# a1q123456/image_stitching

Hardware: AMD Instinct MI355X
Metric: 4K frames stitched/sec (higher is better)
Workload: dtype u8

## Files before the change

### image_stitching_amd/csrc/homography.h

```cpp
#pragma once
#include "common.h"

struct HomoCall {
    const float* src;
    const float* dst;
    uint8_t* mask;
    long long pt_off;
    int n;
    int active;
};

struct HomoResult {
    double H[9];
    int ok;
    int iters;
    int ninl;
    int pad;
};

struct HomoBatch {
    int count = 0;
    long long points = 0;
    int max_iters = 0;
    void* mem = nullptr;
    size_t bytes = 0;
    HomoCall* calls = nullptr;
    HomoResult* results = nullptr;
    void* state = nullptr;
    int* sub_idx = nullptr;
    double* Hc = nullptr;
    int* valid = nullptr;
    int* good = nullptr;
    float* scr = nullptr;
    double* rec = nullptr;
    int* draw_idx = nullptr;
    int* fin = nullptr;
    int2* work = nullptr;
    unsigned* work_ctr = nullptr;
};

int homo_batch_reserve(MisContext* ctx, HomoBatch* b, int count, long long points, int max_iters);
int homo_batch_debug_states(MisContext* ctx, const HomoBatch* b, int* out, int cap);
void homo_batch_release(HomoBatch* b);
enum MotionModel { MODEL_HOMOGRAPHY = 0, MODEL_AFFINE_PARTIAL = 1 };
struct HomoParams { double thresh; int max_iters; double confidence; MotionModel model = MODEL_HOMOGRAPHY; int refine_iters = 10; };
struct HomoHooks {
    hipEvent_t after_first_draw = nullptr, after_second_draw = nullptr;
    hipStream_t spec_stream = nullptr;
    hipEvent_t spec_fork = nullptr, spec_join = nullptr, spec_mark = nullptr;
};
enum RansacPhase { PHASE_FIRST = 0, PHASE_SECOND = 1 };
enum TailStep { TAIL_MASK, TAIL_REFINE };
int homo_solve(MisContext* ctx, HomoBatch* b, const HomoParams& prm, hipStream_t stream = nullptr, const HomoHooks* hooks = nullptr);
int homo_phase(MisContext* ctx, HomoBatch* b, const HomoParams& prm, RansacPhase phase, hipStream_t stream, const HomoHooks* hooks = nullptr);
int homo_tails(MisContext* ctx, HomoBatch* b, const HomoParams& prm, RansacPhase phase, TailStep step, hipStream_t stream);
```

### image_stitching_amd/csrc/homography.hip

```cpp
#include "homography.h"
#include "dev_math.h"
#include <algorithm>
#include <mutex>
#include <vector>

namespace {

#ifndef MIS_PHASE0
#define MIS_PHASE0 128
#endif
constexpr int PHASE0 = MIS_PHASE0;
constexpr int RNG_TABLE = 1 << 17;
#ifndef MIS_HQ_HYPS
#define MIS_HQ_HYPS 64
#endif
constexpr int HQ_HYPS = MIS_HQ_HYPS;
constexpr int TB = 256;

struct RansacState {
    int mode;
    int n_sub;
    int iter, niters, max_good, done, best_k;
    int tail_pending;
    int draw_k, draw_fail;
    long long draw_pos;
    int spec_k, spec_fail;
    long long spec_pos;
};
__device__ __forceinline__ void ransac_reset(RansacState* st, const int mode, const int max_iters) {
    st->mode = mode;
    st->n_sub = 0; st->iter = 0; st->niters = max_iters > 1 ? max_iters : 1; st->max_good = 0; st->done = 0; st->best_k = -1; st->tail_pending = 0;
    st->draw_k = 0; st->draw_fail = 0; st->draw_pos = 0;
    st->spec_k = 0; st->spec_fail = 0; st->spec_pos = 0;
}

enum DrawPhase { DRAW_FIRST, DRAW_SECOND, DRAW_SPEC };
enum TailKind {
    TAIL_REPLAY_FINISH,
    TAIL_REPLAY_ONLY,
    TAIL_MASK_ONLY,
    TAIL_REFINE_ONLY,
};

#ifdef MIS_TAIL_PROF
#define PROF_ONLY(...) __VA_ARGS__
__device__ unsigned long long g_draw_prof[12];
__device__ unsigned long long g_hyp_prof[8];
__device__ unsigned long long g_jac_prof[8];
__device__ unsigned long long g_tail_log[6 * 1024];
__device__ unsigned g_tail_log_n;
__device__ unsigned long long g_tail_prof[12];
#else
#define PROF_ONLY(...)
#endif
#if defined(MIS_TAIL_PROF) && defined(MIS_JAC_PROF)
#define JAC_ONLY(...) __VA_ARGS__
#else
#define JAC_ONLY(...)
#endif
#if defined(MIS_TAIL_PROF) && defined(MIS_PS_PROF)
#define PS_ONLY(...) __VA_ARGS__
#else
#define PS_ONLY(...)
#endif
#define PROF_T0(v) PROF_ONLY(unsigned long long v = wall_clock64())
#define PROF_ADD(i, v) PROF_ONLY(do { if (threadIdx.x == 0) atomicAdd(&g_tail_prof[i], wall_clock64() - (v)); } while (0))
#define JP_T(v) JAC_ONLY(const unsigned long long v = __builtin_readcyclecounter())
#define JP_ADD(i, a, b) JAC_ONLY(do { if (threadIdx.x == 0) atomicAdd(&g_jac_prof[i], (b) - (a)); } while (0))
#define JP_KEEP(...) JAC_ONLY(asm volatile("" :: __VA_ARGS__))
#define PS_T(v) PS_ONLY(const unsigned long long v = __builtin_readcyclecounter())
#define PS_SUM(v) PS_ONLY(unsigned long long v = 0)
#define PS_ACC(v, a, b) PS_ONLY(v += (b) - (a))
#define PS_KEEP(x) PS_ONLY(asm volatile("" :: "v"(x)))
#define PS_ADD(i, who, a, b) PS_ONLY(do { if (threadIdx.x == (who)) atomicAdd(&g_jac_prof[i], (b) - (a)); } while (0))
#define PROF_ROTATIONS(S, n) PROF_ONLY(do { if (threadIdx.x == 0) { atomicAdd(&g_tail_prof[1], (unsigned long long)(n)); (S).prof_rot += (n); } } while (0))
#define PROF_LM_ITERATION(S) PROF_ONLY(do { if (threadIdx.x == 0) { atomicAdd(&g_tail_prof[3], 1ull); (S).prof_lm++; } } while (0))
#define PROF_LM_PASS(np) PROF_ONLY(do { if (threadIdx.x == 0) { atomicAdd(&g_jac_prof[6], (unsigned long long)(np)); atomicAdd(&g_jac_prof[7], 1ull); } } while (0))
#define PROF_FIRST_ENTRY(kind, want, wg_in) PROF_ONLY(const unsigned long long wg_in = wall_clock64(); if ((kind) == TAIL_REFINE_ONLY && (want) == 0 && threadIdx.x == 0) atomicMin(&g_tail_prof[8], wg_in))
#define PROF_LAST_EXIT(kind, want, wg_in) PROF_ONLY(do { if ((kind) == TAIL_REFINE_ONLY && (want) == 0 && threadIdx.x == 0) { const unsigned long long o = wall_clock64(); \
        atomicMax(&g_tail_prof[9], o); atomicMax(&g_tail_prof[10], o - (wg_in)); atomicAdd(&g_tail_prof[11], 1ull); } } while (0))
#define PROF_REPLAY(lo, t0) PROF_ONLY(do { if ((lo) > 0) { const unsigned long long d = wall_clock64() - (t0); atomicAdd(&g_hyp_prof[6], d); atomicMax(&g_hyp_prof[7], d); } } while (0))
#define PROF_TAIL_BEGIN(S, pt) PROF_ONLY(unsigned long long pt = wall_clock64(); if (threadIdx.x == 0) { (S).prof_rot = 0; (S).prof_lm = 0; })
#define PROF_TAIL_END(S, np, kind, want, pt) PROF_ONLY(do { if (threadIdx.x == 0) { \
        atomicAdd(&g_tail_prof[5], wall_clock64() - (pt)); atomicAdd(&g_tail_prof[6], 1ull); atomicMax(&g_tail_prof[7], wall_clock64() - (pt)); \
        const int code[4] = {0, 1, 3, 4}; const unsigned k = atomicAdd(&g_tail_log_n, 1u); if (k < 1024) { unsigned long long* e = g_tail_log + 6 * k; e[0] = np; e[1] = (S).prof_lm; e[2] = (S).prof_rot; e[3] = wall_clock64() - (pt); e[4] = code[kind] * 10 + (want); e[5] = pt; } } } while (0))
struct DrawProf {
    PROF_ONLY(unsigned long long t0 = wall_clock64(), last = t0, sim, dbl; int chunks = 0;)
    __device__ __forceinline__ void simulated() { PROF_ONLY(chunks++; sim = wall_clock64();) }
    __device__ __forceinline__ void doubled() { PROF_ONLY(dbl = wall_clock64();) }
    __device__ __forceinline__ void ranked() {
        PROF_ONLY(const unsigned long long now = wall_clock64(); atomicAdd(&g_draw_prof[8], sim - last); atomicAdd(&g_draw_prof[9], dbl - sim); atomicAdd(&g_draw_prof[10], now - dbl); atomicAdd(&g_draw_prof[11], 1ull);)
    }
    __device__ __forceinline__ void chunk_end() { PROF_ONLY(last = wall_clock64();) }
// ... 604 lines not shown
            for (int i = 0; i < n; i++) { double tv = s.e(HQ_V + n * m + i); s.e(HQ_V + n * m + i) = s.e(HQ_V + n * k + i); s.e(HQ_V + n * k + i) = tv; }
        }
        __builtin_amdgcn_fence(__ATOMIC_ACQ_REL, "wavefront");
    }
}

__device__ int dlt4_quad(const float* M, const float* m, const QSlot s, const int q, double* H) {
    const int count = 4;
    double cMx = 0, cMy = 0, cmx = 0, cmy = 0, sMx = 0, sMy = 0, smx = 0, smy = 0;
    for (int i = 0; i < count; i++) { cmx += m[2 * i]; cmy += m[2 * i + 1]; cMx += M[2 * i]; cMy += M[2 * i + 1]; }
    cmx /= count; cmy /= count; cMx /= count; cMy /= count;
    for (int i = 0; i < count; i++) {
        smx += fabs(m[2 * i] - cmx); smy += fabs(m[2 * i + 1] - cmy);
        sMx += fabs(M[2 * i] - cMx); sMy += fabs(M[2 * i + 1] - cMy);
    }
    if (fabs(smx) < DBL_EPSILON || fabs(smy) < DBL_EPSILON || fabs(sMx) < DBL_EPSILON || fabs(sMy) < DBL_EPSILON) return 0;
    smx = count / smx; smy = count / smy; sMx = count / sMx; sMy = count / sMy;
    double LtL[45];
#pragma unroll
    for (int e = 0; e < 45; e++) LtL[e] = 0;
#pragma unroll
    for (int i = 0; i < count; i++) {
        const double x = (m[2 * i] - cmx) * smx, y = (m[2 * i + 1] - cmy) * smy;
        const double X = (M[2 * i] - cMx) * sMx, Y = (M[2 * i + 1] - cMy) * sMy;
        const double Lx[9] = {X, Y, 1, 0, 0, 0, -x * X, -x * Y, -x};
        const double Ly[9] = {0, 0, 0, X, Y, 1, -y * X, -y * Y, -y};
        int e = 0;
#pragma unroll
        for (int j = 0; j < 9; j++)
#pragma unroll
            for (int k = j; k < 9; k++, e++) LtL[e] += Lx[j] * Lx[k] + Ly[j] * Ly[k];
    }
    {
        int e = 0;
#pragma unroll
        for (int j = 0; j < 9; j++)
#pragma unroll
            for (int k = j; k < 9; k++, e++) {
                if ((e & 3) != q) continue;
                if (k == j) s.e(HQ_W + j) = LtL[e];
                else s.e(hq_T(j) + k) = LtL[e];
            }
    }
    __builtin_amdgcn_fence(__ATOMIC_ACQ_REL, "wavefront");
    jacobi9_quad(s, q);
    double H0[9];
    for (int i = 0; i < 9; i++) H0[i] = s.e(HQ_V + 72 + i);
    const double nrm[8] = {cmx, cmy, cMx, cMy, smx, smy, sMx, sMy};
    dlt_denormalise(H0, nrm, H);
    return 1;
}

constexpr int HQ_WG_PER_CU = 2;
constexpr int HC_WG_PER_CU = 4;
constexpr int HC_HYPS = 4;
enum { WL_N = 0, WL_SOLVE = 1, WL_CTRS = 2 };
static_assert(HQ_HYPS % 16 == 0 && HQ_HYPS % HC_HYPS == 0, "a work-list entry splits into whole solve and count tickets");
__device__ __forceinline__ unsigned first_ticket() { return __builtin_amdgcn_readfirstlane(blockIdx.x * (blockDim.x >> 6) + (threadIdx.x >> 6)); }
__device__ __forceinline__ unsigned next_ticket(unsigned* ctr, unsigned tickets) {
    const unsigned waves = gridDim.x * (blockDim.x >> 6);
    if (tickets <= waves) return tickets;
    return waves + __builtin_amdgcn_readfirstlane(atomicAdd(ctr, (threadIdx.x & 63) == 0 ? 1u : 0u));
}

__global__ __launch_bounds__(4 * HQ_HYPS) void hyp_quad_kernel(const HomoCall* calls, const RansacState* states, const int* sub_idx, double* Hc, int* valid,
                                                               int max_iters, const int2* work, unsigned* work_ctr) {
#if MIS_CHAIN_PRIO
    __builtin_amdgcn_s_setprio(MIS_CHAIN_PRIO);
#endif
    extern __shared__ double sl[];
    const int lane = threadIdx.x & 63, q = lane & 3;
    const int h = threadIdx.x >> 2;
    const unsigned tickets = work_ctr[WL_N] * (HQ_HYPS / 16);
    const QSlot s{sl + h};
    for (unsigned tk = first_ticket(); tk < tickets; tk = next_ticket(work_ctr + WL_SOLVE, tickets)) {
        const int2 w = work[tk / (HQ_HYPS / 16)];
        const int b = w.x;
        const RansacState& st = states[b];
        const int limit = min(st.n_sub, st.niters);
        const int k = w.y + (int)(tk % (HQ_HYPS / 16)) * 16 + (lane >> 2);
        if (k < limit) {
            const HomoCall c = calls[b];
            const int* id = sub_idx + ((size_t)b * max_iters + k) * 4;
            float ms1[8], ms2[8];
#pragma unroll
            for (int i = 0; i < 4; i++) {
                int qq = id[i];
                ms1[2 * i] = c.src[2 * qq]; ms1[2 * i + 1] = c.src[2 * qq + 1];
                ms2[2 * i] = c.dst[2 * qq]; ms2[2 * i + 1] = c.dst[2 * qq + 1];
            }
            double H[9];
            const int ok = dlt4_quad(ms1, ms2, s, q, H);
            if (ok) {
                double* o = Hc + ((size_t)b * max_iters + k) * 9;
#pragma unroll
                for (int i = 0; i < 9; i++) o[i] = H[i];
            }
            valid[(size_t)b * max_iters + k] = ok;
        }
    }
}

constexpr int HC_UNROLL = 4;
__global__ __launch_bounds__(256) void hyp_count_kernel(const HomoCall* calls, const RansacState* states, const double* Hc, const int* valid, int* good,
                                                        int max_iters, float thr, const int2* work, const unsigned* work_ctr) {
    const int lane = threadIdx.x & 63;
    const unsigned tickets = work_ctr[WL_N] * (HQ_HYPS / HC_HYPS), waves = gridDim.x * (blockDim.x >> 6);
    for (unsigned tk = first_ticket(); tk < tickets; tk += waves) {
        const int2 w = work[tk / (HQ_HYPS / HC_HYPS)];
        const int b = w.x;
        const RansacState& st = states[b];
        const int limit = min(st.n_sub, st.niters);
        const int k0 = w.y + (int)(tk % (HQ_HYPS / HC_HYPS)) * HC_HYPS;
        if (k0 >= limit) continue;
        const size_t e0 = (size_t)b * max_iters + k0;
        float Hf[HC_HYPS][9];
        bool use[HC_HYPS];
        int cnt[HC_HYPS];
#pragma unroll
        for (int j = 0; j < HC_HYPS; j++) {
            use[j] = k0 + j < limit && valid[e0 + j];
            cnt[j] = 0;
#pragma unroll
            for (int i = 0; i < 9; i++) Hf[j][i] = use[j] ? (float)Hc[(e0 + j) * 9 + i] : 0.f;
        }
        const HomoCall c = calls[b];
        const float2* src = reinterpret_cast<const float2*>(c.src);
        const float2* dst = reinterpret_cast<const float2*>(c.dst);
        for (int i0 = 0; i0 < c.n; i0 += 64 * HC_UNROLL) {
            float2 M[HC_UNROLL], m[HC_UNROLL];
            bool in[HC_UNROLL];
#pragma unroll
            for (int u = 0; u < HC_UNROLL; u++) {
                const int i = i0 + 64 * u + lane;
                in[u] = i < c.n;
                M[u] = src[min(i, c.n - 1)]; m[u] = dst[min(i, c.n - 1)];
            }
#pragma unroll
            for (int u = 0; u < HC_UNROLL; u++)
#pragma unroll
                for (int j = 0; j < HC_HYPS; j++)
                    if (use[j]) cnt[j] += __popcll(__ballot(in[u] && is_inlier(Hf[j], M[u].x, M[u].y, m[u].x, m[u].y, thr)));
        }
#pragma unroll
        for (int j = 0; j < HC_HYPS; j++) if (k0 + j < limit) good[e0 + j] = cnt[j];
    }
}

#ifndef MIS_PS_PTS
#define MIS_PS_PTS 32
#endif
constexpr int PS_PTS = MIS_PS_PTS;
constexpr int PS_TERMS = 42;
constexpr int PS_PITCH = 43;
constexpr int PS_STAGE = PS_PTS * PS_PITCH;
constexpr size_t TAIL_DYN_LDS = sizeof(double) * 2 * PS_STAGE;
struct TailShared {
    double A[81], V[81], W[9];
    double best[9], nrm[8];
    double lm[8 + 8 + 64 + 64 + 8 + 8 + 8 + 8];
    float Hf[9];
    int indR[9], indC[9];
    int np, go;
    int bad;
    double chunk[TB * 10];
    int staged;
    int done_now;
    int base, wcnt[TB / 64];
    PROF_ONLY(int prof_rot, prof_lm;)
};
__device__ __forceinline__ float4 tail_load_point(const float* s1, const float* d1, int i) {
    const float2 dd = reinterpret_cast<const float2*>(d1)[i], ss = reinterpret_cast<const float2*>(s1)[i];
    return make_float4(dd.x, dd.y, ss.x, ss.y);
}
__device__ __forceinline__ void lds_barrier() { mis_lds_barrier(); }

__device__ __forceinline__ void wave_sync() {
    __builtin_amdgcn_fence(__ATOMIC_ACQ_REL, "wavefront");
    __builtin_amdgcn_wave_barrier();
}
__device__ __forceinline__ double jc_readlane(double v, int lane) {
    return __hiloint2double(__builtin_amdgcn_readlane(__double2hiint(v), lane), __builtin_amdgcn_readlane(__double2loint(v), lane));
}
template <int CTRL, int ROW_MASK = 0xf>
__device__ __forceinline__ double jc_max_step(double v) {
    const int hi = __double2hiint(v), lo = __double2loint(v);
    const int ohi = ROW_MASK == 0xf ? 0 : hi, olo = ROW_MASK == 0xf ? 0 : lo;
    const double o = __hiloint2double(__builtin_amdgcn_update_dpp(ohi, hi, CTRL, ROW_MASK, 0xf, false), __builtin_amdgcn_update_dpp(olo, lo, CTRL, ROW_MASK, 0xf, false));
    double r;
    asm("v_max_f64 %0, %1, %2" : "=v"(r) : "v"(v), "v"(o));
    return r;
}
__device__ __forceinline__ double jc_row_max(double v) {
    v = jc_max_step<0xB1>(v);
    v = jc_max_step<0x4E>(v);
    v = jc_max_step<0x141>(v);
    v = jc_max_step<0x140>(v);
    return v;
// ... 605 lines not shown
template <bool AFFINE = false>
__device__ __forceinline__ void mask_and_compact(TailShared& S, const TailProblem& p, const float thr) {
    const int t = threadIdx.x, n = p.n;
    const HomoCall& c = p.c;
    for (int i0 = 0; i0 < n; i0 += TB) {
        int i = i0 + t, f = 0;
        if (i < n) f = AFFINE ? aff_is_inlier(S.Hf, c.src[2 * i], c.src[2 * i + 1], c.dst[2 * i], c.dst[2 * i + 1], thr)
                              : is_inlier(S.Hf, c.src[2 * i], c.src[2 * i + 1], c.dst[2 * i], c.dst[2 * i + 1], thr);
        if (c.mask && i < n) c.mask[i] = (uint8_t)f;
        unsigned long long bal = __ballot(f);
        int within = __popcll(bal & ((1ull << (t & 63)) - 1ull));
        if ((t & 63) == 0) S.wcnt[t >> 6] = __popcll(bal);
        __syncthreads();
        int off = S.base;
        for (int k = 0; k < (t >> 6); k++) off += S.wcnt[k];
        if (f) {
            p.s1[2 * (off + within)] = c.src[2 * i]; p.s1[2 * (off + within) + 1] = c.src[2 * i + 1];
            p.d1[2 * (off + within)] = c.dst[2 * i]; p.d1[2 * (off + within) + 1] = c.dst[2 * i + 1];
        }
        __syncthreads();
        if (t == 0) { int s = 0; for (int k = 0; k < TB / 64; k++) s += S.wcnt[k]; S.base += s; }
        __syncthreads();
    }
}

__device__ __forceinline__ void refine_on_inliers(TailShared& S, const TailProblem& p, const int np, const TailKind kind, const int want) {
    const int t = threadIdx.x;
    PROF_TAIL_BEGIN(S, pt);
    if (np > 0) {
        const float4 pt0 = t < np ? tail_load_point(p.s1, p.d1, t) : make_float4(0.f, 0.f, 0.f, 0.f);
        dlt_coop(S, p.s1, p.d1, np, pt0, p.rec);
        PROF_ADD(4, pt);
        lm_refine_coop(S, p.s1, p.d1, np, pt0, p.rec);
    }
    PROF_TAIL_END(S, np, kind, want, pt);
}

template <class Model>
__device__ __forceinline__ void tail_problem(TailShared& S, const Model& m, const HomoCall* calls, RansacState* states, const int* valid, const int* good, float* scr_all,
                                             HomoResult* results, int lo, int hi, int max_iters, double confidence, float thr, int* fin, TailKind kind, int want, unsigned* work_ctr) {
    if (work_ctr && blockIdx.x == 0 && threadIdx.x < WL_CTRS) work_ctr[threadIdx.x] = 0;
#if MIS_CHAIN_PRIO
    __builtin_amdgcn_s_setprio(MIS_CHAIN_PRIO);
#endif
    if (threadIdx.x == 0) { S.staged = m.staged; S.bad = 0; }
    m.reset_stages();
    __syncthreads();
    const int b = blockIdx.x, t = threadIdx.x;
    TailProblem p;
    p.b = b; p.c = calls[b]; p.n = p.c.n; p.st = states + b; p.res = results + b;
    p.s1 = scr_all + 4 * p.c.pt_off; p.d1 = p.s1 + 2 * (size_t)(p.n > 0 ? p.n : 0); p.rec = m.rec(p.c);
    RansacState* const st = p.st;
    const bool refines = kind == TAIL_REFINE_ONLY;
    if (kind == TAIL_MASK_ONLY || refines) {
        if (st->tail_pending != (refines ? 2 : 1) || fin[b] != want) return;
        __syncthreads();
    } else {
        if (st->done) return;
        const int mode = st->mode;
        if (t == 0) S.done_now = 0;
        __syncthreads();
        if (mode != 2) { m.no_loop(S, p, mode, lo, fin); return; }
        replay_hypotheses<Model::MODEL_POINTS>(S, p, valid, good, lo, hi, max_iters, confidence, fin);
        __syncthreads();
        if (!S.done_now) return;
        if (kind == TAIL_REPLAY_ONLY) { if (t == 0) st->tail_pending = 1; return; }
    }
    const int result = st->max_good > 0;
    if (!refines && t == 0) { p.res->iters = st->iter; p.res->ok = result; p.res->ninl = 0; }
    if (!result) {
        for (int i = t; p.c.mask && i < p.n; i += TB) p.c.mask[i] = 0;
        if (t == 0) st->tail_pending = 0;
        return;
    }
    if (t == 0) { m.load_best(S, p, max_iters); S.base = refines ? p.res->ninl : 0; }
    __syncthreads();
    if (!refines) mask_and_compact<Model::AFFINE>(S, p, thr);
    const int np = S.base;
    if (kind == TAIL_MASK_ONLY) {
        if (t == 0) { p.res->ninl = np; m.store(p.res, S.best); st->tail_pending = 2; }
        return;
    }
    m.refine(S, p, np, kind, want);
    if (t == 0) { m.store(p.res, S.best); p.res->ninl = np; if (refines) st->tail_pending = 0; }
}

struct HomographyTail {
    static constexpr int MODEL_POINTS = 4;
    static constexpr bool AFFINE = false;
    const double* Hc; double* rec_all; int staged;
    PROF_ONLY(unsigned long long wg_in;)
    __device__ __forceinline__ void reset_stages() const {
        if (staged)
            for (int i = threadIdx.x; i < 2 * PS_PTS; i += TB) tail_dyn[i * PS_PITCH + PS_TERMS] = 0.;
    }
    __device__ __forceinline__ double* rec(const HomoCall& c) const { return rec_all + 10 * c.pt_off; }
    __device__ __forceinline__ void no_loop(TailShared& S, const TailProblem& p, const int mode, const int lo, int* fin) const { finish_without_loop(S, p, mode, lo, fin); }
    __device__ __forceinline__ void load_best(TailShared& S, const TailProblem& p, const int max_iters) const {
        const double* hb = Hc + ((size_t)p.b * max_iters + p.st->best_k) * 9;
        for (int i = 0; i < 9; i++) { S.best[i] = hb[i]; S.Hf[i] = (float)hb[i]; }
    }
    __device__ __forceinline__ void refine(TailShared& S, const TailProblem& p, const int np, const TailKind kind, const int want) const {
        refine_on_inliers(S, p, np, kind, want);
        PROF_LAST_EXIT(kind, want, wg_in);
    }
    __device__ __forceinline__ void store(HomoResult* res, const double* best) const { for (int i = 0; i < 9; i++) res->H[i] = best[i]; }
};
__global__ __launch_bounds__(TB) __attribute__((amdgpu_waves_per_eu(MIS_TAIL_WAVES, 8))) void scan_tail_kernel(const HomoCall* calls, RansacState* states, const double* Hc, const int* valid, const int* good,
                                                       float* scr_all, double* rec_all, HomoResult* results, int lo, int hi, int max_iters,
                                                       double confidence, float thr, int* fin, TailKind kind, int want, int staged, unsigned* work_ctr) {
    PROF_FIRST_ENTRY(kind, want, wg_in);
    __shared__ TailShared S;
    tail_problem(S, HomographyTail{Hc, rec_all, staged PROF_ONLY(, wg_in)}, calls, states, valid, good, scr_all, results, lo, hi, max_iters, confidence, thr, fin, kind, want, work_ctr);
}


__device__ __forceinline__ void aff_hypothesis(const float2 p1, const float2 P1, const float2 p2, const float2 P2, double* M) {
    const double x1 = p1.x, y1 = p1.y, X1 = P1.x, Y1 = P1.y, x2 = p2.x, y2 = p2.y, X2 = P2.x, Y2 = P2.y;
    const double d = 1. / ((x1 - x2) * (x1 - x2) + (y1 - y2) * (y1 - y2));
    const double S0 = d * ((X1 - X2) * (x1 - x2) + (Y1 - Y2) * (y1 - y2));
    const double S1 = d * ((Y1 - Y2) * (x1 - x2) - (X1 - X2) * (y1 - y2));
    const double S2 = d * ((Y1 - Y2) * (x1 * y2 - x2 * y1) - (X1 * y2 - X2 * y1) * (y1 - y2) - (X1 * x2 - X2 * x1) * (x1 - x2));
    const double S3 = d * (-(X1 - X2) * (x1 * y2 - x2 * y1) - (Y1 * x2 - Y2 * x1) * (x1 - x2) - (Y1 * y2 - Y2 * y1) * (y1 - y2));
    M[0] = S0; M[1] = -S1; M[2] = S2; M[3] = S1; M[4] = S0; M[5] = S3;
}
__device__ __forceinline__ void aff_hypothesis_of(const HomoCall& c, const int* id, double* M) {
    const float2* src = reinterpret_cast<const float2*>(c.src);
    const float2* dst = reinterpret_cast<const float2*>(c.dst);
    aff_hypothesis(src[id[0]], dst[id[0]], src[id[1]], dst[id[1]], M);
}

constexpr int AD_CHUNK = 4096;
constexpr int AD_PER = AD_CHUNK / TB;
// ... 328 lines not shown
    }
    return n;
}

void homo_batch_release(HomoBatch* b) {
    if (b->mem) hipFree(b->mem);
    b->mem = nullptr; b->bytes = 0;
}

namespace {

struct Engine {
    MisContext* ctx; HomoBatch* b; hipStream_t st; RngTable rt; HomoHooks hk;
    int max_iters, p0; double confidence; float thr;
    bool affine; int lm_iters;
    static constexpr size_t hq_lds = sizeof(double) * HQ_ELEMS * HQ_STRIDE;

    int open(MisContext* ctx_, HomoBatch* b_, const HomoParams& prm, hipStream_t stream, const HomoHooks* hooks) {
        ctx = ctx_; b = b_; hk = hooks ? *hooks : HomoHooks();
        MIS_CHECK(ctx, prm.max_iters >= 1 && prm.max_iters <= b->max_iters, MIS_E_INVALID, "max_iters %d outside the reserved range", prm.max_iters);
        MIS_CHECK(ctx, prm.confidence > 0 && prm.confidence < 1, MIS_E_INVALID, "confidence must be in (0,1)");
        MIS_CHECK(ctx, prm.model == MODEL_HOMOGRAPHY || prm.model == MODEL_AFFINE_PARTIAL, MIS_E_UNSUPPORTED, "unknown motion model %d", (int)prm.model);
        MIS_CHECK(ctx, prm.refine_iters >= 0, MIS_E_INVALID, "refine_iters must be >= 0");
        affine = prm.model == MODEL_AFFINE_PARTIAL; lm_iters = prm.refine_iters;
        if (int rc = rng_table(ctx, &rt); rc != MIS_OK) return rc;
        const double thresh = prm.thresh <= 0 ? 3 : prm.thresh;
        thr = (float)(thresh * thresh);
        max_iters = prm.max_iters; p0 = std::min(PHASE0, max_iters); confidence = prm.confidence;
        st = stream ? stream : ctx->stream;
        static bool attr_set[64] = {false};
        if (!attr_set[ctx->device & 63]) {
            MIS_HIP(ctx, hipFuncSetAttribute((const void*)hyp_quad_kernel, hipFuncAttributeMaxDynamicSharedMemorySize, (int)hq_lds));
            attr_set[ctx->device & 63] = true;
        }
        return MIS_OK;
    }
    int close(int rc) const { if (rc == MIS_OK) MIS_HIP(ctx, hipGetLastError()); return rc; }
    void draw(DrawPhase phase, hipStream_t s) const {
        if (affine) {
            hipLaunchKernelGGL(aff_draw_kernel, dim3(b->count), dim3(TB), 0, s, b->calls, (RansacState*)b->state, b->sub_idx, rt.U, rt.state_T, max_iters, phase,
                               phase == DRAW_FIRST ? p0 : max_iters, b->work, b->work_ctr);
            return;
        }
        hipLaunchKernelGGL(draw_kernel, dim3(b->count), dim3(DRAW_TB), 0, s, b->calls, (RansacState*)b->state, b->sub_idx, b->draw_idx, rt.U, rt.state_T, max_iters, phase,
                           phase == DRAW_FIRST ? p0 : max_iters, b->work, b->work_ctr, confidence);
    }
    void hypotheses() const {
        const int ncu = std::max(ctx->num_cu, 1);
        if (affine) {
            hipLaunchKernelGGL(aff_score_kernel, dim3(AH_WG_PER_CU * ncu), dim3(256), 0, st, b->calls, (RansacState*)b->state, (const int*)b->sub_idx, b->valid, b->good,
                               max_iters, thr, (const int2*)b->work, (const unsigned*)b->work_ctr);
            return;
        }
        hipLaunchKernelGGL(hyp_quad_kernel, dim3(HQ_WG_PER_CU * ncu), dim3(4 * HQ_HYPS), hq_lds, st, b->calls, (RansacState*)b->state, b->sub_idx, b->Hc, b->valid, max_iters,
                           (const int2*)b->work, b->work_ctr);
        hipLaunchKernelGGL(hyp_count_kernel, dim3(HC_WG_PER_CU * ncu), dim3(256), 0, st, b->calls, (RansacState*)b->state, (const double*)b->Hc, (const int*)b->valid, b->good,
                           max_iters, thr, (const int2*)b->work, b->work_ctr);
    }
    void scan_tail(TailKind kind, RansacPhase phase) const {
        static const bool plain = getenv("MIS_TAIL_PLAIN") != nullptr && atoi(getenv("MIS_TAIL_PLAIN")) != 0;
        const int staged = (kind == TAIL_REPLAY_ONLY || kind == TAIL_MASK_ONLY || plain) ? 0 : 1;
        const bool replay = kind == TAIL_REPLAY_FINISH || kind == TAIL_REPLAY_ONLY, second = phase == PHASE_SECOND;
        const int lo = replay && second ? p0 : 0, hi = replay && second ? max_iters : p0, want = !replay && second ? 1 : 0;
        if (affine) {
            hipLaunchKernelGGL(aff_tail_kernel, dim3(b->count), dim3(TB), 0, st, b->calls, (RansacState*)b->state, (const int*)b->sub_idx, (const int*)b->valid,
                               (const int*)b->good, b->scr, b->results, lo, hi, max_iters, confidence, thr, b->fin, kind, want, lm_iters, replay ? b->work_ctr : nullptr);
            return;
        }
        hipLaunchKernelGGL(scan_tail_kernel, dim3(b->count), dim3(TB), staged ? TAIL_DYN_LDS : (size_t)0, st, b->calls, (RansacState*)b->state, b->Hc, b->valid, b->good, b->scr,
                           b->rec, b->results, lo, hi, max_iters, confidence, thr, b->fin, kind, want, staged, replay ? b->work_ctr : nullptr);
    }
    int run_phase(RansacPhase ph, TailKind replay) const {
        if (ph == PHASE_FIRST) {
            MIS_HIP(ctx, hipMemsetAsync(b->fin, 0xff, sizeof(int) * (size_t)b->count, st));
            draw(DRAW_FIRST, st);
            if (hk.after_first_draw) MIS_HIP(ctx, hipEventRecord(hk.after_first_draw, st));
            if (hk.spec_stream && max_iters > p0 && !affine) {
                MIS_HIP(ctx, hipEventRecord(hk.spec_fork, st));
                MIS_HIP(ctx, hipStreamWaitEvent(hk.spec_stream, hk.spec_fork, 0));
                draw(DRAW_SPEC, hk.spec_stream);
                MIS_HIP(ctx, hipEventRecord(hk.spec_join, hk.spec_stream));
                if (hk.spec_mark) MIS_HIP(ctx, hipEventRecord(hk.spec_mark, hk.spec_stream));
            }
        } else {
            if (max_iters <= p0) return MIS_OK;
            if (hk.spec_stream && !affine) MIS_HIP(ctx, hipStreamWaitEvent(st, hk.spec_join, 0));
            draw(DRAW_SECOND, st);
            if (hk.after_second_draw) MIS_HIP(ctx, hipEventRecord(hk.after_second_draw, st));
        }
        hypotheses();
        scan_tail(replay, ph);
        return MIS_OK;
    }
};

}

int homo_solve(MisContext* ctx, HomoBatch* b, const HomoParams& prm, hipStream_t stream, const HomoHooks* hooks) {
    Engine e;
    int rc = e.open(ctx, b, prm, stream, hooks);
    if (rc == MIS_OK) rc = e.run_phase(PHASE_FIRST, TAIL_REPLAY_FINISH);
    if (rc == MIS_OK) rc = e.run_phase(PHASE_SECOND, TAIL_REPLAY_FINISH);
    return e.close(rc);
}

int homo_phase(MisContext* ctx, HomoBatch* b, const HomoParams& prm, RansacPhase phase, hipStream_t stream, const HomoHooks* hooks) {
    Engine e;
    int rc = e.open(ctx, b, prm, stream, hooks);
    if (rc == MIS_OK) rc = e.run_phase(phase, TAIL_REPLAY_ONLY);
    return e.close(rc);
}

int homo_tails(MisContext* ctx, HomoBatch* b, const HomoParams& prm, RansacPhase phase, TailStep step, hipStream_t stream) {
    Engine e;
    const int rc = e.open(ctx, b, prm, stream, nullptr);
    if (rc == MIS_OK) e.scan_tail(step == TAIL_MASK ? TAIL_MASK_ONLY : TAIL_REFINE_ONLY, phase);
    return e.close(rc);
}
```

### image_stitching_amd/csrc/match.hip

```cpp
#include "common.h"
#include <thread>
#include <chrono>
#include <atomic>
#include "dev_math.h"
#include "homography.h"
#include <algorithm>
#include <vector>

namespace {

struct FeatDev {
    const uint8_t* desc;
    const MisKeyPoint* kps;
    int n, w, h;
};

#include "knn_plan.h"

constexpr int KNN_TILE = 256;
__global__ __launch_bounds__(256) void knn2_hamming_kernel(const FeatDev* feats, const PairDesc* pairs, int* idx2, float* dist2) {
    __shared__ uint4 tr[KNN_TILE * 2];
    const PairDesc pd = pairs[blockIdx.y >> 1];
    const bool fwd = (blockIdx.y & 1) == 0;
    const FeatDev Q = feats[fwd ? pd.i : pd.j], T = feats[fwd ? pd.j : pd.i];
// ... 732 lines not shown
};
int carve_pinned(MisContext* ctx, Arena& arena, const MatchPlan& pl, MatchPinned* h) {
    const size_t n = pl.fd.size(), np = pl.pairs.size(), mt = pl.m_total;
    auto lay = [&](Carver c) {
        h->feats = (FeatDev*)c.at(sizeof(FeatDev) * n); h->pairs = (PairDesc*)c.at(sizeof(PairDesc) * np); h->frames = (HmFrame*)c.at(sizeof(HmFrame) * n);
        h->jobs = (HmJob*)c.at(sizeof(HmJob) * pl.hm_jobs.size()); h->nm = (int*)c.at(sizeof(int) * np); h->out = (PairOut*)c.at(sizeof(PairOut) * np);
        h->r1 = (HomoResult*)c.at(sizeof(HomoResult) * np); h->r2 = (HomoResult*)c.at(sizeof(HomoResult) * np); h->r3 = (HomoResult*)c.at(sizeof(HomoResult) * np);
        h->fin = (int*)c.at(sizeof(int) * np); h->m = (MisDMatch*)c.at(sizeof(MisDMatch) * mt); h->mask = (uint8_t*)c.at(mt); h->l2_bad = (volatile int*)c.at(sizeof(int));
        return c.off;
    };
    MIS_HIP(ctx, arena.reserve(lay(Carver{})));
    lay(Carver{(uintptr_t)arena.p});
    return MIS_OK;
}

int enqueue_knn(MisContext* ctx, MatchWorkspace* ws, const MatchPlan& pl, const MisFeatures* feats, const MatchDev& d, const MatchPinned& h) {
    hipStream_t st = ctx->stream;
    const int n = (int)pl.fd.size(), np = (int)pl.pairs.size();
    if (pl.kind == DESC_L2) return l2_knn2_pairs(ctx, ws->l2, feats, n, pl.pairs.data(), np, true, d.idx, d.dist, (int*)h.l2_bad);
    if (pl.maxq > HM_MAX_TRAINS) {
        hipLaunchKernelGGL(knn2_hamming_kernel, dim3((pl.maxq + 255) / 256, 2 * np), dim3(256), 0, st, (const FeatDev*)d.feats, (const PairDesc*)d.pairs, d.idx, d.dist);
        return MIS_OK;
    }
    Carver lc;
    const size_t o_fr = lc.take(sizeof(HmFrame) * n), o_jobs = lc.take(sizeof(HmJob) * pl.hm_jobs.size());
    for (int i = 0; i < n; i++) {
        const size_t rows = (size_t)(std::max(feats[i].n, 1) + HM_ROWPAD - 1) / HM_ROWPAD * HM_ROWPAD;
        h.frames[i].train_off = lc.take(rows * 128); h.frames[i].query_off = lc.take(rows * 128);
    }
    MIS_HIP(ctx, ws->l2.reserve(lc.off));
    uint8_t* L = (uint8_t*)ws->l2.p;
    MIS_HIP(ctx, hipMemcpyAsync(L + o_fr, h.frames, sizeof(HmFrame) * n, hipMemcpyHostToDevice, st));
    const int maxpad = (pl.maxq + HM_ROWPAD - 1) / HM_ROWPAD * HM_ROWPAD;
    hipLaunchKernelGGL(hamming_expand4_kernel, dim3(maxpad * 8 / 256, n), dim3(256), 0, st, (const FeatDev*)d.feats, (const HmFrame*)(L + o_fr), (int8_t*)L);
    memcpy(h.jobs, pl.hm_jobs.data(), sizeof(HmJob) * pl.hm_jobs.size());
    MIS_HIP(ctx, hipMemcpyAsync(L + o_jobs, h.jobs, sizeof(HmJob) * pl.hm_jobs.size(), hipMemcpyHostToDevice, st));
    hipLaunchKernelGGL(knn2_hamming_fp4_kernel, dim3((unsigned)pl.hm_jobs.size()), dim3(256), 0, st, (const FeatDev*)d.feats, (const PairDesc*)d.pairs,
                       (const HmFrame*)(L + o_fr), (const int8_t*)L, d.idx, d.dist, (const HmJob*)(L + o_jobs));
    return MIS_OK;
}

int enqueue_chains(MisContext* ctx, MatchWorkspace* ws, int np, const MisMatchParams* p, int model, const MatchDev& d, const MatchPinned& h) {
    hipStream_t st = ctx->stream;
    int rc;
    if (!ws->side && (rc = mis_aux_stream(ctx, 0, &ws->side)) != MIS_OK) return rc;
    trace_mark(ws, 0, st);
    if (!ws->third && (rc = mis_aux_stream(ctx, 1, &ws->third)) != MIS_OK) return rc;
    MIS_HIP(ctx, hipEventRecord(ws->ev_matches.ev, st));
    MIS_HIP(ctx, hipStreamWaitEvent(ws->third, ws->ev_matches.ev, 0));
    hipLaunchKernelGGL(pack_lists_kernel, dim3(np), dim3(256), 0, ws->third, (const PairDesc*)d.pairs, np, (const int*)d.nm, (const MisDMatch*)d.matches, h.m, h.nm);
    MIS_HIP(ctx, hipEventRecord(ws->ev_lists.ev, ws->third));
    if (model == MIS_MATCH_AFFINE_PARTIAL) {
        const HomoParams aprm{p->ransac_thresh, p->max_iters, p->confidence, MODEL_AFFINE_PARTIAL, 10};
        for (RansacPhase ph : {PHASE_FIRST, PHASE_SECOND})
            if ((rc = homo_phase(ctx, &ws->b1, aprm, ph, st)) != MIS_OK || (rc = homo_tails(ctx, &ws->b1, aprm, ph, TAIL_MASK, st)) != MIS_OK ||
                (rc = homo_tails(ctx, &ws->b1, aprm, ph, TAIL_REFINE, st)) != MIS_OK) return rc;
        MIS_HIP(ctx, hipStreamWaitEvent(st, ws->ev_lists.ev, 0));
        return MIS_OK;
    }
    const HomoParams prm{p->ransac_thresh, p->max_iters, p->confidence};
    HomoHooks chain;
    chain.spec_stream = ws->side; chain.spec_fork = ws->ev_spec_fork.ev; chain.spec_join = ws->ev_spec_join.ev;
    if (match_trace() && ws->tev[8].ready(hipEventDefault) == hipSuccess) chain.spec_mark = ws->tev[8].ev;
    if (match_trace() && ws->tev[7].ready(hipEventDefault) == hipSuccess) chain.after_second_draw = ws->tev[7].ev;
    if ((rc = homo_phase(ctx, &ws->b1, prm, PHASE_FIRST, st, &chain)) != MIS_OK || (rc = homo_tails(ctx, &ws->b1, prm, PHASE_FIRST, TAIL_MASK, st)) != MIS_OK) return rc;
    MIS_HIP(ctx, hipEventRecord(ws->ev_phase0.ev, st));
    trace_mark(ws, 1, st);
    MIS_HIP(ctx, hipStreamWaitEvent(ws->side, ws->ev_phase0.ev, 0));
    hipLaunchKernelGGL(second_calls_kernel, dim3((np + 127) / 128), dim3(128), 0, ws->side, np, (const HomoCall*)ws->b1.calls, (const HomoResult*)ws->b1.results,
                       (const float*)ws->b1.scr, (const int*)ws->b1.fin, PHASE_FIRST, p->num_matches_thresh2, ws->b2.calls, d.out);
    HomoHooks gate;
    gate.after_first_draw = ws->ev_gate = ws->ev_draw1.ev;
    if ((rc = homo_solve(ctx, &ws->b2, prm, ws->side, &gate)) != MIS_OK) return rc;
    MIS_HIP(ctx, hipEventRecord(ws->ev_side_done.ev, ws->side));
    trace_mark(ws, 4, ws->side);
    MIS_HIP(ctx, hipStreamWaitEvent(ws->third, ws->ev_phase0.ev, 0));
    if ((rc = homo_tails(ctx, &ws->b1, prm, PHASE_FIRST, TAIL_REFINE, ws->third)) != MIS_OK) return rc;
    trace_mark(ws, 6, ws->third);
    if ((rc = homo_phase(ctx, &ws->b1, prm, PHASE_SECOND, st, &chain)) != MIS_OK || (rc = homo_tails(ctx, &ws->b1, prm, PHASE_SECOND, TAIL_MASK, st)) != MIS_OK) return rc;
    MIS_HIP(ctx, hipEventRecord(ws->ev_phase1.ev, st));
    trace_mark(ws, 2, st);
    if ((rc = homo_tails(ctx, &ws->b1, prm, PHASE_SECOND, TAIL_REFINE, st)) != MIS_OK) return rc;
    trace_mark(ws, 3, st);
    MIS_HIP(ctx, hipStreamWaitEvent(ws->third, ws->ev_phase1.ev, 0));
    hipLaunchKernelGGL(second_calls_kernel, dim3((np + 127) / 128), dim3(128), 0, ws->third, np, (const HomoCall*)ws->b1.calls, (const HomoResult*)ws->b1.results,
                       (const float*)ws->b1.scr, (const int*)ws->b1.fin, PHASE_SECOND, p->num_matches_thresh2, ws->b3.calls, d.out);
    if ((rc = homo_solve(ctx, &ws->b3, prm, ws->third)) != MIS_OK) return rc;
    MIS_HIP(ctx, hipEventRecord(ws->ev_third_done.ev, ws->third));
    trace_mark(ws, 5, ws->third);
    MIS_HIP(ctx, hipStreamWaitEvent(st, ws->ev_third_done.ev, 0));
    MIS_HIP(ctx, hipStreamWaitEvent(st, ws->ev_side_done.ev, 0));
    return MIS_OK;
}

void enqueue_results(MatchWorkspace* ws, int np, size_t m_total, const MatchDev& d, const MatchPinned& h, hipStream_t st, int model) {
    CopySegs cs{};
    const void* srcs[6] = {d.out, ws->b1.results, ws->b2.results, ws->b3.results, ws->b1.fin, d.mask};
    void* dsts[6] = {h.out, h.r1, h.r2, h.r3, h.fin, h.mask};
    const size_t sizes[6] = {sizeof(PairOut) * np, sizeof(HomoResult) * np, sizeof(HomoResult) * np, sizeof(HomoResult) * np, sizeof(int) * np, m_total};
    cs.n = 6;
    for (int k = 0; k < 6; k++) { cs.src[k] = (const uint8_t*)srcs[k]; cs.dst[k] = (uint8_t*)dsts[k]; cs.bytes[k] = model == MIS_MATCH_AFFINE_PARTIAL && (k == 2 || k == 3) ? 0u : (unsigned)sizes[k]; }
    hipLaunchKernelGGL(copy_segments_kernel, dim3(64), dim3(256), 0, st, cs);
}

int assemble_matches(MisContext* ctx, MatchWorkspace* ws, const MatchPlan& pl, const MatchPinned& h, int n, int model, MisMatchesInfo* out,
                     std::chrono::steady_clock::time_point* ts) {
    const int np = (int)pl.pairs.size();
    auto drop_lists = [&]() {
        for (const PairDesc& pd : pl.pairs)
            for (MisMatchesInfo* m : {&out[pd.i * n + pd.j], &out[pd.j * n + pd.i]}) { free(m->matches); free(m->inliers_mask); init_info(m); }
    };
    MIS_HIP(ctx, hipEventSynchronize(ws->ev_lists.ev));
    size_t packed_off = 0;
    for (int k = 0; k < np; k++) {
        const PairDesc& pd = pl.pairs[k];
        MisMatchesInfo *a = &out[pd.i * n + pd.j], *b = &out[pd.j * n + pd.i];
        const int nm = h.nm[k];
        a->src_img_idx = pd.i; a->dst_img_idx = pd.j;
        a->n_matches = nm;
        a->matches = (MisDMatch*)malloc(sizeof(MisDMatch) * (size_t)(nm + 1));
        memcpy(a->matches, h.m + packed_off, sizeof(MisDMatch) * (size_t)nm);
        packed_off += (size_t)nm;
        b->matches = (MisDMatch*)malloc(sizeof(MisDMatch) * (size_t)(nm + 1));
        for (int q = 0; q < nm; q++) { b->matches[q] = a->matches[q]; std::swap(b->matches[q].query_idx, b->matches[q].train_idx); }
    }
    const hipError_t e = hipStreamSynchronize(ctx->stream);
    ws->drained = e == hipSuccess;
    *ts = std::chrono::steady_clock::now();
    if (e != hipSuccess || *h.l2_bad) {
        drop_lists();
        if (e != hipSuccess) return mis_set_error(ctx, MIS_E_HIP, "hipStreamSynchronize failed: %s (%s:%d)", hipGetErrorString(e), __FILE__, __LINE__);
        return mis_set_error(ctx, MIS_E_UNSUPPORTED, "L2 matching needs integer-valued descriptors in 0..255 (SIFT style)");
    }
    for (int k = 0; k < np; k++) {
        const PairDesc& pd = pl.pairs[k];
// ... 450 lines not shown
```

Before: 3535.

## Fuse inlier counting into hypothesis solve and merge replay with mask tail

```diff
diff --git a/image_stitching_amd/csrc/homography.h b/image_stitching_amd/csrc/homography.h
--- a/image_stitching_amd/csrc/homography.h
+++ b/image_stitching_amd/csrc/homography.h
@@ -50,7 +50,6 @@
     hipEvent_t spec_fork = nullptr, spec_join = nullptr, spec_mark = nullptr;
 };
 enum RansacPhase { PHASE_FIRST = 0, PHASE_SECOND = 1 };
-enum TailStep { TAIL_MASK, TAIL_REFINE };
 int homo_solve(MisContext* ctx, HomoBatch* b, const HomoParams& prm, hipStream_t stream = nullptr, const HomoHooks* hooks = nullptr);
 int homo_phase(MisContext* ctx, HomoBatch* b, const HomoParams& prm, RansacPhase phase, hipStream_t stream, const HomoHooks* hooks = nullptr);
-int homo_tails(MisContext* ctx, HomoBatch* b, const HomoParams& prm, RansacPhase phase, TailStep step, hipStream_t stream);
+int homo_tails(MisContext* ctx, HomoBatch* b, const HomoParams& prm, RansacPhase phase, hipStream_t stream);
diff --git a/image_stitching_amd/csrc/homography.hip b/image_stitching_amd/csrc/homography.hip
--- a/image_stitching_amd/csrc/homography.hip
+++ b/image_stitching_amd/csrc/homography.hip
@@ -37,8 +37,7 @@
 enum DrawPhase { DRAW_FIRST, DRAW_SECOND, DRAW_SPEC };
 enum TailKind {
     TAIL_REPLAY_FINISH,
-    TAIL_REPLAY_ONLY,
-    TAIL_MASK_ONLY,
+    TAIL_REPLAY_MASK,
     TAIL_REFINE_ONLY,
 };
 
@@ -749,10 +748,8 @@
 }
 
 constexpr int HQ_WG_PER_CU = 2;
-constexpr int HC_WG_PER_CU = 4;
-constexpr int HC_HYPS = 4;
 enum { WL_N = 0, WL_SOLVE = 1, WL_CTRS = 2 };
-static_assert(HQ_HYPS % 16 == 0 && HQ_HYPS % HC_HYPS == 0, "a work-list entry splits into whole solve and count tickets");
+static_assert(HQ_HYPS % 16 == 0, "a work-list entry splits into whole tickets");
 __device__ __forceinline__ unsigned first_ticket() { return __builtin_amdgcn_readfirstlane(blockIdx.x * (blockDim.x >> 6) + (threadIdx.x >> 6)); }
 __device__ __forceinline__ unsigned next_ticket(unsigned* ctr, unsigned tickets) {
     const unsigned waves = gridDim.x * (blockDim.x >> 6);
@@ -760,8 +757,29 @@
     return waves + __builtin_amdgcn_readfirstlane(atomicAdd(ctr, (threadIdx.x & 63) == 0 ? 1u : 0u));
 }
 
-__global__ __launch_bounds__(4 * HQ_HYPS) void hyp_quad_kernel(const HomoCall* calls, const RansacState* states, const int* sub_idx, double* Hc, int* valid,
-                                                               int max_iters, const int2* work, unsigned* work_ctr) {
+constexpr int HQ_COUNT_UNROLL = 8;
+__device__ __forceinline__ int count_inliers_quad(const float* Hf, const HomoCall& c, const int q, const float thr) {
+    const float2* src = reinterpret_cast<const float2*>(c.src);
+    const float2* dst = reinterpret_cast<const float2*>(c.dst);
+    int cnt = 0;
+    for (int i0 = 0; i0 < c.n; i0 += 4 * HQ_COUNT_UNROLL) {
+        float2 M[HQ_COUNT_UNROLL], m[HQ_COUNT_UNROLL];
+#pragma unroll
+        for (int u = 0; u < HQ_COUNT_UNROLL; u++) {
+            const int i = min(i0 + 4 * u + q, c.n - 1);
+            M[u] = src[i]; m[u] = dst[i];
+        }
+#pragma unroll
+        for (int u = 0; u < HQ_COUNT_UNROLL; u++)
+            cnt += (i0 + 4 * u + q < c.n) & is_inlier(Hf, M[u].x, M[u].y, m[u].x, m[u].y, thr);
+    }
+    cnt += __builtin_amdgcn_update_dpp(0, cnt, 0xB1, 0xf, 0xf, false);
+    cnt += __builtin_amdgcn_update_dpp(0, cnt, 0x4E, 0xf, 0xf, false);
+    return cnt;
+}
+
+__global__ __launch_bounds__(4 * HQ_HYPS) void hyp_quad_kernel(const HomoCall* calls, const RansacState* states, const int* sub_idx, double* Hc, int* valid, int* good,
+                                                               int max_iters, float thr, const int2* work, unsigned* work_ctr) {
 #if MIS_CHAIN_PRIO
     __builtin_amdgcn_s_setprio(MIS_CHAIN_PRIO);
 #endif
@@ -788,59 +806,17 @@
             }
             double H[9];
             const int ok = dlt4_quad(ms1, ms2, s, q, H);
+            int cnt = 0;
             if (ok) {
                 double* o = Hc + ((size_t)b * max_iters + k) * 9;
-#pragma unroll
-                for (int i = 0; i < 9; i++) o[i] = H[i];
+                float Hf[9];
+#pragma unroll
+                for (int i = 0; i < 9; i++) { o[i] = H[i]; Hf[i] = (float)H[i]; }
+                cnt = count_inliers_quad(Hf, c, q, thr);
             }
             valid[(size_t)b * max_iters + k] = ok;
-        }
-    }
-}
-
-constexpr int HC_UNROLL = 4;
-__global__ __launch_bounds__(256) void hyp_count_kernel(const HomoCall* calls, const RansacState* states, const double* Hc, const int* valid, int* good,
-                                                        int max_iters, float thr, const int2* work, const unsigned* work_ctr) {
-    const int lane = threadIdx.x & 63;
-    const unsigned tickets = work_ctr[WL_N] * (HQ_HYPS / HC_HYPS), waves = gridDim.x * (blockDim.x >> 6);
-    for (unsigned tk = first_ticket(); tk < tickets; tk += waves) {
-        const int2 w = work[tk / (HQ_HYPS / HC_HYPS)];
-        const int b = w.x;
-        const RansacState& st = states[b];
-        const int limit = min(st.n_sub, st.niters);
-        const int k0 = w.y + (int)(tk % (HQ_HYPS / HC_HYPS)) * HC_HYPS;
-        if (k0 >= limit) continue;
-        const size_t e0 = (size_t)b * max_iters + k0;
-        float Hf[HC_HYPS][9];
-        bool use[HC_HYPS];
-        int cnt[HC_HYPS];
-#pragma unroll
-        for (int j = 0; j < HC_HYPS; j++) {
-            use[j] = k0 + j < limit && valid[e0 + j];
-            cnt[j] = 0;
-#pragma unroll
-            for (int i = 0; i < 9; i++) Hf[j][i] = use[j] ? (float)Hc[(e0 + j) * 9 + i] : 0.f;
-        }
-        const HomoCall c = calls[b];
-        const float2* src = reinterpret_cast<const float2*>(c.src);
-        const float2* dst = reinterpret_cast<const float2*>(c.dst);
-        for (int i0 = 0; i0 < c.n; i0 += 64 * HC_UNROLL) {
-            float2 M[HC_UNROLL], m[HC_UNROLL];
-            bool in[HC_UNROLL];
-#pragma unroll
-            for (int u = 0; u < HC_UNROLL; u++) {
-                const int i = i0 + 64 * u + lane;
-                in[u] = i < c.n;
-                M[u] = src[min(i, c.n - 1)]; m[u] = dst[min(i, c.n - 1)];
-            }
-#pragma unroll
-            for (int u = 0; u < HC_UNROLL; u++)
-#pragma unroll
-                for (int j = 0; j < HC_HYPS; j++)
-                    if (use[j]) cnt[j] += __popcll(__ballot(in[u] && is_inlier(Hf[j], M[u].x, M[u].y, m[u].x, m[u].y, thr)));
-        }
-#pragma unroll
-        for (int j = 0; j < HC_HYPS; j++) if (k0 + j < limit) good[e0 + j] = cnt[j];
+            good[(size_t)b * max_iters + k] = cnt;
+        }
     }
 }
 
@@ -1552,8 +1528,8 @@
     p.s1 = scr_all + 4 * p.c.pt_off; p.d1 = p.s1 + 2 * (size_t)(p.n > 0 ? p.n : 0); p.rec = m.rec(p.c);
     RansacState* const st = p.st;
     const bool refines = kind == TAIL_REFINE_ONLY;
-    if (kind == TAIL_MASK_ONLY || refines) {
-        if (st->tail_pending != (refines ? 2 : 1) || fin[b] != want) return;
+    if (refines) {
+        if (!st->tail_pending || fin[b] != want) return;
         __syncthreads();
     } else {
         if (st->done) return;
@@ -1564,7 +1540,6 @@
         replay_hypotheses<Model::MODEL_POINTS>(S, p, valid, good, lo, hi, max_iters, confidence, fin);
         __syncthreads();
         if (!S.done_now) return;
-        if (kind == TAIL_REPLAY_ONLY) { if (t == 0) st->tail_pending = 1; return; }
     }
     const int result = st->max_good > 0;
     if (!refines && t == 0) { p.res->iters = st->iter; p.res->ok = result; p.res->ninl = 0; }
@@ -1577,8 +1552,8 @@
     __syncthreads();
     if (!refines) mask_and_compact<Model::AFFINE>(S, p, thr);
     const int np = S.base;
-    if (kind == TAIL_MASK_ONLY) {
-        if (t == 0) { p.res->ninl = np; m.store(p.res, S.best); st->tail_pending = 2; }
+    if (kind == TAIL_REPLAY_MASK) {
+        if (t == 0) { p.res->ninl = np; m.store(p.res, S.best); st->tail_pending = 1; }
         return;
     }
     m.refine(S, p, np, kind, want);
@@ -2013,15 +1988,13 @@
                                max_iters, thr, (const int2*)b->work, (const unsigned*)b->work_ctr);
             return;
         }
-        hipLaunchKernelGGL(hyp_quad_kernel, dim3(HQ_WG_PER_CU * ncu), dim3(4 * HQ_HYPS), hq_lds, st, b->calls, (RansacState*)b->state, b->sub_idx, b->Hc, b->valid, max_iters,
-                           (const int2*)b->work, b->work_ctr);
-        hipLaunchKernelGGL(hyp_count_kernel, dim3(HC_WG_PER_CU * ncu), dim3(256), 0, st, b->calls, (RansacState*)b->state, (const double*)b->Hc, (const int*)b->valid, b->good,
+        hipLaunchKernelGGL(hyp_quad_kernel, dim3(HQ_WG_PER_CU * ncu), dim3(4 * HQ_HYPS), hq_lds, st, b->calls, (RansacState*)b->state, b->sub_idx, b->Hc, b->valid, b->good,
                            max_iters, thr, (const int2*)b->work, b->work_ctr);
     }
     void scan_tail(TailKind kind, RansacPhase phase) const {
         static const bool plain = getenv("MIS_TAIL_PLAIN") != nullptr && atoi(getenv("MIS_TAIL_PLAIN")) != 0;
-        const int staged = (kind == TAIL_REPLAY_ONLY || kind == TAIL_MASK_ONLY || plain) ? 0 : 1;
-        const bool replay = kind == TAIL_REPLAY_FINISH || kind == TAIL_REPLAY_ONLY, second = phase == PHASE_SECOND;
+        const int staged = (kind == TAIL_REPLAY_MASK || plain) ? 0 : 1;
+        const bool replay = kind != TAIL_REFINE_ONLY, second = phase == PHASE_SECOND;
         const int lo = replay && second ? p0 : 0, hi = replay && second ? max_iters : p0, want = !replay && second ? 1 : 0;
         if (affine) {
             hipLaunchKernelGGL(aff_tail_kernel, dim3(b->count), dim3(TB), 0, st, b->calls, (RansacState*)b->state, (const int*)b->sub_idx, (const int*)b->valid,
@@ -2068,13 +2041,13 @@
 int homo_phase(MisContext* ctx, HomoBatch* b, const HomoParams& prm, RansacPhase phase, hipStream_t stream, const HomoHooks* hooks) {
     Engine e;
     int rc = e.open(ctx, b, prm, stream, hooks);
-    if (rc == MIS_OK) rc = e.run_phase(phase, TAIL_REPLAY_ONLY);
+    if (rc == MIS_OK) rc = e.run_phase(phase, TAIL_REPLAY_MASK);
     return e.close(rc);
 }
 
-int homo_tails(MisContext* ctx, HomoBatch* b, const HomoParams& prm, RansacPhase phase, TailStep step, hipStream_t stream) {
+int homo_tails(MisContext* ctx, HomoBatch* b, const HomoParams& prm, RansacPhase phase, hipStream_t stream) {
     Engine e;
     const int rc = e.open(ctx, b, prm, stream, nullptr);
-    if (rc == MIS_OK) e.scan_tail(step == TAIL_MASK ? TAIL_MASK_ONLY : TAIL_REFINE_ONLY, phase);
+    if (rc == MIS_OK) e.scan_tail(TAIL_REFINE_ONLY, phase);
     return e.close(rc);
 }
diff --git a/image_stitching_amd/csrc/match.hip b/image_stitching_amd/csrc/match.hip
--- a/image_stitching_amd/csrc/match.hip
+++ b/image_stitching_amd/csrc/match.hip
@@ -808,9 +808,7 @@
     MIS_HIP(ctx, hipEventRecord(ws->ev_lists.ev, ws->third));
     if (model == MIS_MATCH_AFFINE_PARTIAL) {
         const HomoParams aprm{p->ransac_thresh, p->max_iters, p->confidence, MODEL_AFFINE_PARTIAL, 10};
-        for (RansacPhase ph : {PHASE_FIRST, PHASE_SECOND})
-            if ((rc = homo_phase(ctx, &ws->b1, aprm, ph, st)) != MIS_OK || (rc = homo_tails(ctx, &ws->b1, aprm, ph, TAIL_MASK, st)) != MIS_OK ||
-                (rc = homo_tails(ctx, &ws->b1, aprm, ph, TAIL_REFINE, st)) != MIS_OK) return rc;
+        if ((rc = homo_solve(ctx, &ws->b1, aprm, st)) != MIS_OK) return rc;
         MIS_HIP(ctx, hipStreamWaitEvent(st, ws->ev_lists.ev, 0));
         return MIS_OK;
     }
@@ -819,7 +817,7 @@
     chain.spec_stream = ws->side; chain.spec_fork = ws->ev_spec_fork.ev; chain.spec_join = ws->ev_spec_join.ev;
     if (match_trace() && ws->tev[8].ready(hipEventDefault) == hipSuccess) chain.spec_mark = ws->tev[8].ev;
     if (match_trace() && ws->tev[7].ready(hipEventDefault) == hipSuccess) chain.after_second_draw = ws->tev[7].ev;
-    if ((rc = homo_phase(ctx, &ws->b1, prm, PHASE_FIRST, st, &chain)) != MIS_OK || (rc = homo_tails(ctx, &ws->b1, prm, PHASE_FIRST, TAIL_MASK, st)) != MIS_OK) return rc;
+    if ((rc = homo_phase(ctx, &ws->b1, prm, PHASE_FIRST, st, &chain)) != MIS_OK) return rc;
     MIS_HIP(ctx, hipEventRecord(ws->ev_phase0.ev, st));
     trace_mark(ws, 1, st);
     MIS_HIP(ctx, hipStreamWaitEvent(ws->side, ws->ev_phase0.ev, 0));
@@ -831,12 +829,12 @@
     MIS_HIP(ctx, hipEventRecord(ws->ev_side_done.ev, ws->side));
     trace_mark(ws, 4, ws->side);
     MIS_HIP(ctx, hipStreamWaitEvent(ws->third, ws->ev_phase0.ev, 0));
-    if ((rc = homo_tails(ctx, &ws->b1, prm, PHASE_FIRST, TAIL_REFINE, ws->third)) != MIS_OK) return rc;
+    if ((rc = homo_tails(ctx, &ws->b1, prm, PHASE_FIRST, ws->third)) != MIS_OK) return rc;
     trace_mark(ws, 6, ws->third);
-    if ((rc = homo_phase(ctx, &ws->b1, prm, PHASE_SECOND, st, &chain)) != MIS_OK || (rc = homo_tails(ctx, &ws->b1, prm, PHASE_SECOND, TAIL_MASK, st)) != MIS_OK) return rc;
+    if ((rc = homo_phase(ctx, &ws->b1, prm, PHASE_SECOND, st, &chain)) != MIS_OK) return rc;
     MIS_HIP(ctx, hipEventRecord(ws->ev_phase1.ev, st));
     trace_mark(ws, 2, st);
-    if ((rc = homo_tails(ctx, &ws->b1, prm, PHASE_SECOND, TAIL_REFINE, st)) != MIS_OK) return rc;
+    if ((rc = homo_tails(ctx, &ws->b1, prm, PHASE_SECOND, st)) != MIS_OK) return rc;
     trace_mark(ws, 3, st);
     MIS_HIP(ctx, hipStreamWaitEvent(ws->third, ws->ev_phase1.ev, 0));
     hipLaunchKernelGGL(second_calls_kernel, dim3((np + 127) / 128), dim3(128), 0, ws->third, np, (const HomoCall*)ws->b1.calls, (const HomoResult*)ws->b1.results,
```

Result: no change. 3505 (-0.8%).
